# Kirkice/3DGaussian

Measured on AMD Instinct MI355X. Metric: Mpixels/sec fwd+bwd @1M Gaussians 800×800; PSNR vs torch ref, higher is better.
Workload: dtype f32 (splat contractions on v_mfma_f32_32x32x16_f16 with f32 accumulation; every operand in two round-to-nearest f16 pieces, pre-scaled into f16's normal range, three piece products: <= 3*2^-22 per product, forward and backward; no-depth-gradient mode)

## Files before the change

3dgaussian_amd/csrc/gr_hip.hip:

```cpp

#include <hip/hip_runtime.h>
#include <hipcub/hipcub.hpp>
#include <rocprim/rocprim.hpp>

#include <cmath>
#include <cstdint>
#include <cstdio>
#include <cstdlib>
#include <cstring>
#include <atomic>
#include <mutex>
#include <string>
#include <vector>

#include "../../include/gr_hip.h"

#ifndef GR_TAIL2
#define GR_TAIL2 1
#endif
#ifndef GR_DEBUG_PREP_REPS
#define GR_DEBUG_PREP_REPS 1
#endif
#ifndef GR_DEBUG_BIN_REPS
#define GR_DEBUG_BIN_REPS 1
#endif
#ifndef GR_DEBUG_SKIP
#define GR_DEBUG_SKIP 0
#endif

#define GR_VERSION_STR "gr_hip 0.1.0 (gfx950)"

namespace {

thread_local std::string g_last_error;

gr_status set_error(gr_status st, const std::string& msg) {
  g_last_error = msg;
  return st;
}

#define GR_HIP_TRY(expr)                                                                          \
  do {                                                                                            \
    hipError_t e_ = (expr);                                                                       \
    if (e_ != hipSuccess)                                                                         \
      return set_error(GR_ERR_HIP, std::string("HIP error: ") + hipGetErrorString(e_) + " (" +   \
// ... 190 lines not shown
  const float lox = (float)(tx * v.T) + 0.5f, hix = (float)xe + 0.5f;
  const float cx = px < lox ? lox : (px > hix ? hix : px);
  const float dx = cx - px;
  return (dx * dx) * qx;
}
__device__ __forceinline__ float tile_ey(const ViewK& v, float py, float qy, int ty) {
  const int ye = min(ty * v.T + v.T - 1, v.H - 1);
  const float loy = (float)(ty * v.T) + 0.5f, hiy = (float)ye + 0.5f;
  const float cy = py < loy ? loy : (py > hiy ? hiy : py);
  const float dy = cy - py;
  return (dy * dy) * qy;
}
__device__ __forceinline__ int tile_class_e(float e, float thr_cut, float thr_core) {
  return !(e >= thr_cut) ? 0 : (e >= thr_core ? 2 : 1);
}

__device__ __forceinline__ bool tile_pass(const ViewK& v, float px, float py, float qx, float qy, int tx, int ty) {
  return tile_emax(v, px, py, qx, qy, tx, ty) >= radius_thr(v.cutoff);
}

__device__ __forceinline__ int tile_class(const ViewK& v, float px, float py, float qx, float qy, int tx, int ty) {
  const float e = tile_emax(v, px, py, qx, qy, tx, ty);
  if (!(e >= radius_thr(v.cutoff))) return 0;
  return e >= radius_thr(v.core) ? 2 : 1;
}

__device__ __forceinline__ float qcoef(float s) { return (-0.5f * LOG2E) / (s * s); }


constexpr int REC4 = 2;
// ... 298 lines not shown
template <int CD>
__device__ __forceinline__ unsigned long long preprocess_vals(const ViewK& v, int i, float mx, float my, float mz, float s0,
                                                              float s1, const float* __restrict__ col, float op,
                                                              const Geom& g) {
  Proj p;
  project(v, mx, my, mz, s0, s1, p);
  float c[3];
  eval_color<CD>(v, mx, my, mz, col, c);
  int4 r;
  const float qx = qcoef(p.sx);
  const float qy = qcoef(p.sy);
  int core = 0, tail = 0;
  const int area = tile_rect(v, p, op, r);
  if (area > 0) {
    const float thr_cut = radius_thr(v.cutoff), thr_core = radius_thr(v.core);
    for (int ty = r.y; ty <= r.w; ++ty) {
      const float ey = tile_ey(v, p.py, qy, ty);
      for (int tx = r.x; tx <= r.z; ++tx) {
        const int cls = tile_class_e(tile_ex(v, p.px, qx, tx) + ey, thr_cut, thr_core);
        core += cls == 2;
        tail += cls == 1;
      }
    }
  }
  float4* rec = g.rec + (size_t)REC4 * i;
  rec[0] = make_float4(p.px, p.py, qx, qy);
  rec[1] = make_float4(op < 0.0f ? 0.0f : op, clamp01(c[0]), clamp01(c[1]), clamp01(c[2]));
  g.zr[i] = p.za;
  g.rect[i] = r;
  g.counts[i] = (unsigned long long)core | ((unsigned long long)tail << 32);
  return (unsigned long long)core | ((unsigned long long)tail << 32);
}

template <int CD>
__device__ __forceinline__ unsigned long long preprocess_one(const ViewK& v, int i, const float* __restrict__ means,
                                                             const float* __restrict__ scales,
// ... 180 lines not shown
  const Cnt2 cn{i < n ? counts[i].v : 0ull};
  const Cnt2 cb{bsum[b]};
  const int Kc = (int)offsets[n].c();
  const int4 rc = i < n ? rect[i] : make_int4(0, 0, -1, -1);
  const float4 a = i < n ? rec[(size_t)REC4 * i] : make_float4(0.f, 0.f, 0.f, 0.f);
  unsigned long long tot;
  const unsigned long long ex = block_exclusive_scan<4>(cn.v, wsum, tot);
  const int c0 = (int)cb.c(), t0 = (int)cb.t();
  const int nc = (int)(tot & 0xffffffffull), nt = (int)(tot >> 32);
  const bool staged = nc + nt <= EWIN_BLK;
  const unsigned long long run = cb.v + ex;
  if (i < n) offsets[i].v = run;
  if (cn.v != 0) {
    int kc = (int)(run & 0xffffffffull), kt = (int)(run >> 32);
    const float thr_cut = radius_thr(v.cutoff), thr_core = radius_thr(v.core);
    for (int ty = rc.y; ty <= rc.w; ++ty) {
      const float ey = tile_ey(v, a.y, a.w, ty);
      for (int tx = rc.x; tx <= rc.z; ++tx) {
        const int cls = tile_class_e(tile_ex(v, a.x, a.z, tx) + ey, thr_cut, thr_core);
        if (cls == 0) continue;
        const int t = ty * v.tiles_x + tx;
        const int e = cls == 2 ? kc++ - c0 : nc + (kt++ - t0);
        if (staged) {
          sK[e] = (uint16_t)t;
          sI[e] = i;
        } else {
          const int k = e < nc ? c0 + e : Kc + t0 + (e - nc);
          keys[k] = (uint16_t)t;
          ids[k] = i;
        }
      }
    }
  }
  if (!staged) return;
  __syncthreads();
  for (int e = tid; e < nc + nt; e += 256) {
    const int k = e < nc ? c0 + e : Kc + t0 + (e - nc);
    keys[k] = sK[e];
    ids[k] = sI[e];
  }
}
__global__ __launch_bounds__(256) void k_emit_offsets(ViewK v, int n, const int4* __restrict__ rect, const Cnt2* __restrict__ counts,
                                                      const unsigned long long* __restrict__ bsum, Cnt2* __restrict__ offsets,
                                                      const float4* __restrict__ rec, uint16_t* __restrict__ keys,
// ... 658 lines not shown
#ifndef GR_FWD_F16
#define GR_FWD_F16 1
#endif
#ifndef GR_F16_SA
#define GR_F16_SA 4
#endif
#ifndef GR_F16_SB
#define GR_F16_SB 12
#endif
__device__ __forceinline__ int f16_sa_of(float omax) {
  if (!(omax <= 3.0e38f)) return GR_F16_SA;
  int e = 0;
  (void)frexpf(omax, &e);
  return GR_F16_SA - (e > 11 ? e - 11 : 0);
}
__device__ __forceinline__ float f16_resid_lo(float x, unsigned h) {
  float r;
  asm("v_fma_mix_f32 %0, -%1, 1.0, %2 op_sel_hi:[1,0,0]" : "=v"(r) : "v"(h), "v"(x));
  return r;
}
__device__ __forceinline__ float f16_resid_hi(float x, unsigned h) {
  float r;
  asm("v_fma_mix_f32 %0, -%1, 1.0, %2 op_sel:[1,0,0] op_sel_hi:[1,0,0]" : "=v"(r) : "v"(h), "v"(x));
  return r;
}
typedef _Float16 f16x2h_t __attribute__((ext_vector_type(2)));
__device__ __forceinline__ unsigned pk_f16(float a, float b) {
  return __builtin_bit_cast(unsigned, __builtin_convertvector(f32x2_t{a, b}, f16x2h_t));
}
__device__ __forceinline__ void split2h_frag2(const f32x2_t (&v)[4], s16x8 (&f)[2]) {
  unsigned h[4], l[4];
#pragma unroll
  for (int p = 0; p < 4; ++p) {
    h[p] = pk_f16(v[p].x, v[p].y);
    l[p] = pk_f16(f16_resid_lo(v[p].x, h[p]), f16_resid_hi(v[p].y, h[p]));
  }
  f[0] = as_frag(make_uint4(h[0], h[1], h[2], h[3]));
  f[1] = as_frag(make_uint4(l[0], l[1], l[2], l[3]));
}
__device__ __forceinline__ void split2h_frag(const float (&v)[8], s16x8 (&f)[2]) {
  unsigned h[4], l[4];
#pragma unroll
  for (int p = 0; p < 4; ++p) {
    h[p] = pk_f16(v[2 * p], v[2 * p + 1]);
    l[p] = pk_f16(f16_resid_lo(v[2 * p], h[p]), f16_resid_hi(v[2 * p + 1], h[p]));
  }
  f[0] = as_frag(make_uint4(h[0], h[1], h[2], h[3]));
  f[1] = as_frag(make_uint4(l[0], l[1], l[2], l[3]));
}
__device__ __forceinline__ int f16_exp_of(float m) {
  if (!(m > 0.0f) || !(m <= 3.0e38f)) return 0;
  int e = 0;
  (void)frexpf(m, &e);
  return 14 - e;
}
typedef _Float16 f16x8_t __attribute__((ext_vector_type(8)));
__device__ __forceinline__ f32x4 mfma16h(const s16x8& a, const s16x8& b, f32x4 c) {
  return __builtin_amdgcn_mfma_f32_16x16x32_f16(__builtin_bit_cast(f16x8_t, a), __builtin_bit_cast(f16x8_t, b), c, 0, 0, 0);
}
__device__ __forceinline__ f32x4 mfma16h_split2(const s16x8 (&a)[2], const s16x8 (&b)[2], f32x4 c) {
  c = mfma16h(a[1], b[0], c);
  c = mfma16h(a[0], b[1], c);
  return mfma16h(a[0], b[0], c);
// ... 36 lines not shown

template <bool TAIL, bool PRECISE, bool ZCH = true>
__device__ __forceinline__ void fwd_accumulate_bf16(float* smem, int n, int k0, int k1, int tid, int wave, float xc, float yc,
                                                    int gq, const int* __restrict__ pairs, const float4* __restrict__ rec,
                                                    f32x4& cW, f32x4& cR, f32x4& cG, f32x4& cB, f32x4& cD, float sa) {
  constexpr int BUF = FWD_PLANES * TP;
  auto stage = [&](int g, int b) {
    glds4_planes<TAIL, ZCH>(rec_of(g, n, rec), zrec_of(g, n, rec), smem + b * BUF + 64 * wave);
  };
  stage(stage_pair(stage_id(k0 + tid, k1, pairs), k0 + tid, k1), 0);
  int idn = stage_id(k0 + TP + tid, k1, pairs);
  int buf = 0;
  const f32x2_t X = {xc, xc}, Y = {yc, yc};
  constexpr bool F16 = GR_FWD_F16 && !PRECISE && !TAIL && !ZCH;
  const f32x2_t SA = {sa, sa}, SB = {(float)GR_F16_SB, (float)GR_F16_SB};
  (void)SA;
  (void)SB;
  for (int base = k0; base < k1; base += TP, buf ^= 1) {
    stage_wait();
    GR_STAGE_SYNC();
    if (base + TP < k1) stage(stage_pair(idn, base + TP + tid, k1), buf ^ 1);
    idn = stage_id(base + 2 * TP + tid, k1, pairs);
    const int cnt = min(TP, k1 - base) - wave * 64;
    const int nst = cnt <= 0 ? 0 : min(2, (cnt + 31) >> 5);
    for (int st = 0; st < nst; ++st) {
      const float* s = smem + buf * BUF + wave * 64 + st * 32 + 8 * gq;
      auto ld = [&](int f, f32x2_t (&v)[4]) {
        const float4 u0 = *reinterpret_cast<const float4*>(s + f * TP);
        const float4 u1 = *reinterpret_cast<const float4*>(s + f * TP + 4);
        v[0] = f32x2_t{u0.x, u0.y};
        v[1] = f32x2_t{u0.z, u0.w};
        v[2] = f32x2_t{u1.x, u1.y};
// ... 21 lines not shown
        oe[p] = o[p] * ex;
        aW[p] = oe[p];
        if constexpr (ZCH) aD[p] = oe[p] * z[p];
      }
      s16x8 fb[3], f3[3], fb2h[2];
      if constexpr (PRECISE) {
        split3_frag2(bv, fb);
        split3_frag2(aW, f3);
        cW = mfma16_split3(f3, fb, cW);
        if constexpr (ZCH) {
          split3_frag2(aD, f3);
          cD = mfma16_split3(f3, fb, cD);
        }
      } else if (F16) {
        s16x8 f2[2];
        split2h_frag2(bv, fb2h);
        split2h_frag2(aW, f2);
        cW = mfma16h_split2(f2, fb2h, cW);
      } else {
        s16x8 f2b[2], f2[2];
        split2_frag2(bv, f2b);
        fb[0] = f2b[0];
        fb[1] = f2b[1];
        split2_frag2(aW, f2);
        cW = mfma16_split2<false>(f2, fb, cW);
        if constexpr (ZCH) {
          split2_frag2(aD, f2);
          cD = mfma16_split2<false>(f2, fb, cD);
        }
      }
      if constexpr (!TAIL) {
        f32x2_t c[4], a[4];
        s16x8 f2[2];
        if constexpr (F16) {
          ld(5, c);
#pragma unroll
          for (int p = 0; p < 4; ++p) a[p] = oe[p] * c[p];
          split2h_frag2(a, f2);
          cR = mfma16h_split2(f2, fb2h, cR);
          ld(6, c);
#pragma unroll
          for (int p = 0; p < 4; ++p) a[p] = oe[p] * c[p];
          split2h_frag2(a, f2);
          cG = mfma16h_split2(f2, fb2h, cG);
          ld(7, c);
#pragma unroll
          for (int p = 0; p < 4; ++p) a[p] = oe[p] * c[p];
          split2h_frag2(a, f2);
          cB = mfma16h_split2(f2, fb2h, cB);
        } else {
        ld(5, c);
#pragma unroll
        for (int p = 0; p < 4; ++p) a[p] = oe[p] * c[p];
        split2_frag2(a, f2);
        cR = mfma16_split2<PRECISE>(f2, fb, cR);
        ld(6, c);
#pragma unroll
        for (int p = 0; p < 4; ++p) a[p] = oe[p] * c[p];
        split2_frag2(a, f2);
        cG = mfma16_split2<PRECISE>(f2, fb, cG);
        ld(7, c);
#pragma unroll
        for (int p = 0; p < 4; ++p) a[p] = oe[p] * c[p];
// ... 80 lines not shown
      r[0][t] += r[0][t + w];
      r[1][t] += r[1][t + w];
      r[2][t] += r[2][t + w];
    }
    __syncthreads();
  }
  if (t != 0) return;
  float l = (float)(r[0][0] / (double)n1);
  if (n2 > 0) l = l + w_sil * (float)(r[1][0] / (double)n2);
  if (n3 > 0) l = l + w_depth * (float)(r[2][0] / (double)n3);
  *loss = l;
}

__device__ __forceinline__ float sign0(float t) { return t > 0.0f ? 1.0f : (t < 0.0f ? -1.0f : 0.0f); }

template <bool SSIM = false>
__device__ __forceinline__ void pixel_upstream(const ViewK& v, int p, float4 s, float Dp, const float* __restrict__ g_rgb,
                                               const float* __restrict__ g_alpha, const float* __restrict__ g_depth,
                                               const L1Args& l1, float (&u)[5], float& l_rgb, float& l_sil,
                                               const float* g_ssim = nullptr) {
  const float den = 1.0f + s.x, dden = s.x + 1e-6f;
  const float inv = 1.0f / den;
  float gW = 0.f;
  const float C[3] = {s.y, s.z, s.w};
  const float HWf = (float)v.W * (float)v.H;
#pragma unroll
  for (int k = 0; k < 3; ++k) {
    const float r = (view_bg(v, k) + C[k]) * inv;
    float gk;
    if (l1.t_rgb) {
      const float t = clamp01(r) - l1.t_rgb[3 * p + k];
      l_rgb += fabsf(t);
      if constexpr (SSIM)
        gk = sign0(t) * (((1.0f - l1.w_dssim) * l1.g_scale) / (3.0f * HWf)) + g_ssim[k];
      else
        gk = sign0(t) * (l1.g_scale / (3.0f * HWf));
    } else {
      gk = g_rgb[3 * p + k];
    }
    const float go = (r >= 0.0f && r <= 1.0f) ? gk : 0.0f;
    u[k] = go * inv;
    gW -= (go * r) * inv;
  }
  const float al = s.x * inv;
  float ga = 0.0f;
  bool has_a = g_alpha != nullptr;
  if (l1.t_rgb && l1.t_mask) {
    const float t = clamp01(al) - l1.t_mask[p];
    l_sil = fabsf(t);
    ga = sign0(t) * ((l1.w_sil * l1.g_scale) / HWf);
    has_a = true;
  } else if (g_alpha) {
    ga = g_alpha[p];
  }
  if (has_a && al >= 0.0f && al <= 1.0f) gW += ga * (inv * inv);
  const bool dfit = l1.t_rgb && l1.t_depth;
  if (g_depth || dfit) {
    const float d = Dp / dden;
    if (d >= 0.0f) {
      float gd;
      if (dfit) {
        const float M = l1.dscal[0], dm = M + 1e-6f;
        const float t = d / dm - l1.t_depth[p];
        gd = (sign0(t) * ((l1.w_depth * l1.g_scale) / HWf)) / dm;
        if (d == M) gd += l1.dscal[1];
      } else {
        gd = g_depth[p];
      }
      gW -= gd * Dp / (dden * dden);
      u[4] = gd / dden;
    }
  }
  u[3] = gW;
}

__device__ __forceinline__ float saved_depth(const float4* __restrict__ saved4, const float* __restrict__ savedD, int p) {
  const float d = savedD[p] / (saved4[p].x + 1e-6f);
  return d < 0.0f ? 0.0f : d;
}
// ... 187 lines not shown
  }
}

__device__ __forceinline__ void k_pixel_grads_body(ViewK v, const float4* __restrict__ saved4,
                                                     const float* __restrict__ savedD, const float* __restrict__ g_rgb,
                                                     const float* __restrict__ g_alpha, const float* __restrict__ g_depth,
                                                     uint4* __restrict__ UF, int pieces, L1Args l1, bool depth,
                                                     int* __restrict__ ticket, const BI blockIdx, const BI gridDim) {
  const int tile = blockIdx.x, tid = threadIdx.x;
  const int tx = tile % v.tiles_x, ty = tile / v.tiles_x;
  const int x = tx * T + (tid & (T - 1)), y = ty * T + (tid >> 4);
  float u[5] = {0.f, 0.f, 0.f, 0.f, 0.f};
  float l_rgb = 0.f, l_sil = 0.f;
  if (x < v.W && y < v.H) {
    const int p = y * v.W + x;
    pixel_upstream(v, p, saved4[p], savedD[p], g_rgb, g_alpha, g_depth, l1, u, l_rgb, l_sil);
  }
  if (l1.tile_loss) tile_loss_sums(tile, tid, l_rgb, l_sil, l1.tile_loss);
  __shared__ __attribute__((aligned(16))) float sU[6][TP];
  static_assert(sizeof(sU) >= 3 * 256 * sizeof(double), "tile_loss_total scratch");
#pragma unroll
  for (int k = 0; k < 5; ++k) sU[k][tid] = u[k];
  __syncthreads();
  tile_fragments(sU, reinterpret_cast<uint4*>(UF) + (size_t)tile * UF_FRAGS, tid, pieces, depth);
  if (l1.tile_loss && l1.loss_out) {
    __shared__ int last;
    const int tiles = v.tiles_x * v.tiles_y;
    if (arrive_last_tile(ticket, tiles, tile, &last))
      tile_loss_total<true>(l1.tile_loss, tiles, l1.n1, l1.n2, l1.w_sil, l1.t_depth ? l1.n1 / 3 : 0, l1.w_depth,
                            l1.loss_out, reinterpret_cast<double (*)[256]>(&sU[0][0]));
  }
// ... 20 lines not shown
};
__global__ __launch_bounds__(256) void k_pixel_grads_views(VBatch<k_pixel_grads_args> B) {
  const int vb = vbatch_view(B, (int)blockIdx.x);
  const k_pixel_grads_args& a = B.a[vb];
  const int lb = (int)blockIdx.x - B.first[vb], gx = B.gx[vb];
  k_pixel_grads_body(a.v, a.saved4, a.savedD, a.g_rgb, a.g_alpha, a.g_depth, a.UF, a.pieces, a.l1, a.depth, a.ticket, BI{lb % gx, lb / gx}, BI{gx, (B.first[vb + 1] - B.first[vb]) / gx});
}


__device__ __forceinline__ void l1_tile_epilogue(const ViewK& v, int tile, int tid, const float (&acc)[5], bool inside,
                                                 int p, const L1Args& l1, uint4* __restrict__ UF, float* lds,
                                                 bool fragments = true) {
  float u[5] = {0.f, 0.f, 0.f, 0.f, 0.f};
  float l_rgb = 0.f, l_sil = 0.f;
  if (inside)
    pixel_upstream(v, p, make_float4(acc[0], acc[1], acc[2], acc[3]), acc[4], nullptr, nullptr, nullptr, l1, u, l_rgb,
                   l_sil);
  tile_loss_sums(tile, tid, l_rgb, l_sil, l1.tile_loss);
  if (!fragments) return;
  float (*sU)[TP] = reinterpret_cast<float (*)[TP]>(lds);
#pragma unroll
  for (int k = 0; k < 4; ++k) sU[k][tid] = u[k];
  __syncthreads();
  tile_fragments(sU, UF + (size_t)tile * UF_FRAGS, tid, l1.pieces, false);
}

#ifndef GR_FWD_WAVES
#define GR_FWD_WAVES 5
#endif
#ifndef GR_FWD_WAVES3
#define GR_FWD_WAVES3 6
#endif
// ... 440 lines not shown
#define GR_BWD32_PHASE() __builtin_amdgcn_sched_barrier(0)
#else
#define GR_BWD32_PHASE() ((void)0)
#endif
constexpr int F32_PLANES = 8;
constexpr int F32_BUF = F32_PLANES * TP;
constexpr int F32_LD = T32 + 1;
__device__ __forceinline__ f32x16 mfma32h(const s16x8& a, const s16x8& b, f32x16 c) {
  return __builtin_amdgcn_mfma_f32_32x32x16_f16(__builtin_bit_cast(f16x8_t, a), __builtin_bit_cast(f16x8_t, b), c, 0, 0, 0);
}
__device__ __forceinline__ f32x16 mfma32b(const s16x8& a, const s16x8& b, f32x16 c) {
  return __builtin_amdgcn_mfma_f32_32x32x16_bf16(a, b, c, 0, 0, 0);
}
__device__ __forceinline__ constexpr int kslot_off(int j) { return j < 4 ? j : j + 4; }

__device__ __forceinline__ void k_fwd32_l1_body(ViewK v, int n, const int4* __restrict__ items,
                                                                 const int* __restrict__ num_items,
                                                                 const int2* __restrict__ ranges, const int* __restrict__ pairs,
                                                                 const float4* __restrict__ rec, float* __restrict__ fwd_part,
                                                                 float* __restrict__ out_rgb, float* __restrict__ out_alpha,
                                                                 L1Args l1, uint4* __restrict__ UF, const int* __restrict__ f16_sa,
                                                                 const int* __restrict__ tile_item0, int* __restrict__ ticket,
                                                                 int ch, const BI blockIdx, const BI gridDim) {
  __shared__ __attribute__((aligned(16))) float smem[4 * 2 * T32 * F32_LD];
  static_assert(sizeof(smem) >= 2 * F32_BUF * sizeof(float) && sizeof(smem) >= 3 * 256 * sizeof(double), "k_fwd32_l1 LDS");
  __shared__ int last_flag;
  const int nitems = num_items[0], nfull = num_items[1];
  if ((int)blockIdx.x >= nitems) return;
  const int item = (int)blockIdx.x < nfull ? xcd_item(blockIdx.x, nfull) : (int)blockIdx.x;
  const int4 it = items[item];
  const int tile = it.x >> 1, k0 = it.y, k1 = it.z;
  const int tx = tile % v.tiles_x, ty = tile / v.tiles_x;
  const int tid = threadIdx.x, wave = tid >> 6, lane = tid & 63, r = lane & 31, h = lane >> 5;
  const int sa = f16_sa ? *f16_sa : GR_F16_SA;
  f32x16 cW = {}, cR = {}, cG = {}, cB = {};
  if (k1 > k0) {
    auto stage = [&](int g, int b) { glds4_planes<false, false>(rec_of(g, n, rec), nullptr, smem + b * F32_BUF + 64 * wave); };
    stage(stage_pair(stage_id(k0 + tid, k1, pairs), k0 + tid, k1), 0);
    int idn = stage_id(k0 + TP + tid, k1, pairs);
    int buf = 0;
    const float xc = (float)(tx * T32 + r) + 0.5f, yc = (float)(ty * T32 + r) + 0.5f;
    const f32x2_t X = {xc, xc}, Y = {yc, yc}, SA = {(float)sa, (float)sa}, SB = {(float)GR_F16_SB, (float)GR_F16_SB};
    for (int base = k0; base < k1; base += TP, buf ^= 1) {
      stage_wait();
      if (base + TP < k1) stage(stage_pair(idn, base + TP + tid, k1), buf ^ 1);
      idn = stage_id(base + 2 * TP + tid, k1, pairs);
      const int cnt = min(TP, k1 - base) - wave * 64;
      const int nks = cnt <= 0 ? 0 : min(4, (cnt + 15) >> 4);
      for (int ks = 0; ks < nks; ++ks) {
        const float* s = smem + buf * F32_BUF + wave * 64 + ks * 16 + 4 * h;
        auto ld = [&](int f, f32x2_t (&q)[4]) {
          const float4 u0 = *reinterpret_cast<const float4*>(s + f * TP);
          const float4 u1 = *reinterpret_cast<const float4*>(s + f * TP + 8);
          q[0] = f32x2_t{u0.x, u0.y};
          q[1] = f32x2_t{u0.z, u0.w};
          q[2] = f32x2_t{u1.x, u1.y};
          q[3] = f32x2_t{u1.z, u1.w};
        };
        f32x2_t oe[4], bv[4];
        {
          f32x2_t px[4], qx[4], o[4];
          ld(0, px);
          ld(2, qx);
          ld(4, o);
#pragma unroll
          for (int p = 0; p < 4; ++p) {
            const f32x2_t dx = X - px[p];
            const f32x2_t ax = __builtin_elementwise_fma(dx * qx[p], dx, SA);
            const f32x2_t ex = {__builtin_amdgcn_exp2f(ax.x), __builtin_amdgcn_exp2f(ax.y)};
            oe[p] = o[p] * ex;
          }
        }
        __builtin_amdgcn_sched_barrier(0);
        {
          f32x2_t py[4], qy[4];
          ld(1, py);
          ld(3, qy);
#pragma unroll
          for (int p = 0; p < 4; ++p) {
            const f32x2_t dy = Y - py[p];
            const f32x2_t ay = __builtin_elementwise_fma(dy * qy[p], dy, SB);
            bv[p] = f32x2_t{__builtin_amdgcn_exp2f(ay.x), __builtin_amdgcn_exp2f(ay.y)};
          }
        }
        __builtin_amdgcn_sched_barrier(0);
        s16x8 fb[2], fa[2];
        split2h_frag2(bv, fb);
        split2h_frag2(oe, fa);
        cW = mfma32h(fa[1], fb[0], cW);
        cW = mfma32h(fa[0], fb[1], cW);
        cW = mfma32h(fa[0], fb[0], cW);
        f32x2_t c[4], a[4];
#define GR_FWD32_CH(F, ACC)                                   \
  ld(F, c);                                                   \
  _Pragma("unroll") for (int p = 0; p < 4; ++p) a[p] = oe[p] * c[p]; \
  split2h_frag2(a, fa);                                       \
  ACC = mfma32h(fa[1], fb[0], ACC);                           \
  ACC = mfma32h(fa[0], fb[1], ACC);                           \
  ACC = mfma32h(fa[0], fb[0], ACC);
        GR_FWD32_CH(5, cR)
        GR_FWD32_CH(6, cG)
        GR_FWD32_CH(7, cB)
#undef GR_FWD32_CH
      }
    }
    const float sc = __builtin_ldexpf(1.0f, -(sa + GR_F16_SB));
    cW *= sc;
    cR *= sc;
    cG *= sc;
    cB *= sc;
  }
// ... 35 lines not shown
#pragma unroll
      for (int c = 0; c < 4; ++c) acc[q][c] = 0.f;
    for (int e = 0; e < nch; ++e)
#pragma unroll
      for (int q = 0; q < 4; ++q) {
        const float4 pv = ld_through16(src, 4 * 4 * TP32 * e + 16 * (256 * q + tid));
        acc[q][0] += pv.x;
        acc[q][1] += pv.y;
        acc[q][2] += pv.z;
        acc[q][3] += pv.w;
      }
    if (tid == 0) ticket[tile] = 0;
  }
  float u[4][5];
  float l_rgb = 0.f, l_sil = 0.f;
#pragma unroll
  for (int q = 0; q < 4; ++q) {
    const int x = tx * T32 + px0, y = ty * T32 + py0 + 8 * q;
#pragma unroll
    for (int c = 0; c < 5; ++c) u[q][c] = 0.f;
    if (x < v.W && y < v.H && ty >= v.ty0 && ty < v.ty1) {
      const int p = y * v.W + x;
      const float a5[5] = {acc[q][0], acc[q][1], acc[q][2], acc[q][3], 0.0f};
      write_pixel(v, p, a5, out_rgb, out_alpha, nullptr, nullptr, nullptr);
      float lr = 0.f, ls = 0.f;
      pixel_upstream(v, p, make_float4(acc[q][0], acc[q][1], acc[q][2], acc[q][3]), 0.0f, nullptr, nullptr, nullptr, l1,
                     u[q], lr, ls);
      l_rgb += lr;
      l_sil += ls;
    }
  }
  tile_loss_sums(tile, tid, l_rgb, l_sil, l1.tile_loss);
  if (nch > 0) {
    float* sU = smem;
#pragma unroll
    for (int q = 0; q < 4; ++q)
#pragma unroll
      for (int c = 0; c < 4; ++c) sU[c * T32 * F32_LD + px0 * F32_LD + py0 + 8 * q] = u[q][c];
    __syncthreads();
    const float HWf = (float)v.W * (float)v.H, gC = fabsf(l1.g_scale) / (3.0f * HWf);
    const int eC = f16_exp_of(gC), eWb = f16_exp_of(3.0f * gC + fabsf(l1.w_sil * l1.g_scale) / HWf);
    const int ex4[4] = {eC, eC, eC, eWb};
    uint4* fr = UF + (size_t)tile * UF32_STRIDE;
    if (tid == 0) fr[UF32_FRAGS] = make_uint4((unsigned)ex4[0], (unsigned)ex4[1], (unsigned)ex4[2], (unsigned)ex4[3]);
    for (int e = tid; e < 16 * 64; e += 256) {
      const int set = e >> 6, l = e & 63, side = set >> 3, c = (set >> 1) & 3, s = set & 1;
      const int sc = c == 0 ? ex4[0] : (c == 1 ? ex4[1] : (c == 2 ? ex4[2] : ex4[3]));
      float val[8];
      const int m = l & 31, hh = l >> 5;
#pragma unroll
      for (int j = 0; j < 8; ++j) {
        const int k = 16 * s + kslot_pixel(hh, j);
        val[j] = ldexpf(side == 0 ? sU[c * T32 * F32_LD + k * F32_LD + m] : sU[c * T32 * F32_LD + m * F32_LD + k], sc);
      }
      s16x8 f2[2];
      split2h_frag(val, f2);
      __builtin_memcpy(&fr[(set * 2 + 0) * 64 + l], &f2[0], 16);
      __builtin_memcpy(&fr[(set * 2 + 1) * 64 + l], &f2[1], 16);
    }
  }
  const int tiles = v.tiles_x * v.tiles_y;
  if (arrive_last_tile(ticket, tiles, tile, &last_flag))
    tile_loss_total<true>(l1.tile_loss, tiles, l1.n1, l1.n2, l1.w_sil, 0, 0.0f, l1.loss_out,
                          reinterpret_cast<double (*)[256]>(smem));
}
__global__ __launch_bounds__(256, GR_FWD32_WAVES) void k_fwd32_l1(ViewK v, int n, const int4* __restrict__ items,
                                                                 const int* __restrict__ num_items,
                                                                 const int2* __restrict__ ranges, const int* __restrict__ pairs,
                                                                 const float4* __restrict__ rec, float* __restrict__ fwd_part,
                                                                 float* __restrict__ out_rgb, float* __restrict__ out_alpha,
                                                                 L1Args l1, uint4* __restrict__ UF, const int* __restrict__ f16_sa,
// ... 38 lines not shown
  __shared__ __attribute__((aligned(16))) uint4 sUF[2 * 4 * 2 * 2 * 64];
  const int nitems = num_items[1];
  if ((int)blockIdx.x >= nitems) return;
  const int item = xcd_item(blockIdx.x, nitems);
  const int4 it = items[item];
  const int tile = it.x >> 1, k0 = it.y, k1 = it.z;
  if (k1 <= k0) return;
  const int tx = tile % v.tiles_x, ty = tile / v.tiles_x;
  const int tid = threadIdx.x, wave = tid >> 6, lane = tid & 63, r = lane & 31, h = lane >> 5;
  {
    const uint4* src = UF + (size_t)tile * UF32_STRIDE;
    for (int cc = wave; cc < 32; cc += 4) glds16(src + 64 * cc + lane, sUF + 64 * cc);
  }
  const uint4 e4 = UF[(size_t)tile * UF32_STRIDE + UF32_FRAGS];
  const int eC0 = (int)e4.x, eC1 = (int)e4.y, eC2 = (int)e4.z, eW = (int)e4.w;
  const float pxb[2] = {(float)(tx * T32 + 4 * h) + 0.5f, (float)(tx * T32 + 16 + 4 * h) + 0.5f};
  const float pyb[2] = {(float)(ty * T32 + 4 * h) + 0.5f, (float)(ty * T32 + 16 + 4 * h) + 0.5f};
  {
    const int k = k0 + wave * WG + (lane < WG ? lane : 0);
    if (lane < WG) {
      const int gid = stage_pair(stage_id(k, k1, pairs), k, k1);
      glds16(rec_of(gid, n, rec), &sA[0][WG * wave]);
      glds16(rec_of(gid, n, rec) + 1, &sB[0][WG * wave]);
    }
  }
  int idn = stage_id(k0 + NB + wave * WG + (lane < WG ? lane : 0), k1, pairs);
  int buf = 0;
  for (int base = k0; base < k1; base += NB, buf ^= 1) {
    stage_wait();
    if (base == k0) __syncthreads();
// ... 31 lines not shown
      auto contract = [&](int side, int c, const s16x8 (&B)[2][2]) {
        const uint4* A0 = sUF + ((side * 4 + c) * 2 + 0) * 2 * 64;
        f32x16 d = {};
#pragma unroll
        for (int s = 0; s < 2; ++s) d = mfma32h(as_frag(A0[(s * 2 + 1) * 64 + lane]), B[s][0], d);
#pragma unroll
        for (int s = 0; s < 2; ++s) {
          const s16x8 a0 = as_frag(A0[(s * 2) * 64 + lane]);
          d = mfma32h(a0, B[s][1], d);
          d = mfma32h(a0, B[s][0], d);
        }
        return d;
      };
      const float4 bs = make_float4(b.x, ldexpf(b.y, eW - eC0), ldexpf(b.z, eW - eC1), ldexpf(b.w, eW - eC2));
      s16x8 BT[2][2], BR[2][2];
      split2h_frag(ex[0], BT[0]);
      split2h_frag(ex[1], BT[1]);
      float p[16];
      {
        const f32x16 D3 = contract(0, 3, BT);
#pragma unroll
        for (int i = 0; i < 16; ++i) p[i] = D3[i];
      }
      f32x16 Dc = contract(0, 0, BT);
      GR_BWD32_PHASE();
#pragma unroll
      for (int c = 0; c < 3; ++c) {
        const float bc = c == 0 ? bs.y : (c == 1 ? bs.z : bs.w);
        f32x16 Dn;
        if (c < 2) {
          Dn = contract(0, c + 1, BT);
        } else {
          split2h_frag(ey[0], BR[0]);
          split2h_frag(ey[1], BR[1]);
          Dn = contract(1, 3, BR);
        }
#pragma unroll
        for (int i = 0; i < 16; ++i) {
          S[c] = fmaf(ey[i >> 3][i & 7], Dc[i], S[c]);
          p[i] = fmaf(bc, Dc[i], p[i]);
        }
        if (c == 2) {
#pragma unroll
          for (int i = 0; i < 16; ++i) {
            const int s = i >> 3, q = i & 7;
            const float oq = (float)kslot_off(q);
            const float t = ey[s][q] * p[i];
            S4s[s] += t;
            if (q != 0) {
// ... 1206 lines not shown
    }
    sA[0][o] = a0;
    sA[1][o] = a1;
    sA[2][o] = a2;
  }
  __syncthreads();
  float u[5] = {0.f, 0.f, 0.f, 0.f, 0.f};
  float l_rgb = 0.f, l_sil = 0.f;
  if (inside) {
    const float scale = -((l1.w_dssim * l1.g_scale) / (3.0f * ((float)v.W * (float)v.H)));
    const int o = (tid >> 4) * TC + (tid & (T - 1)) * C;
    float gs[3];
#pragma unroll
    for (int k = 0; k < 3; ++k)
      gs[k] = scale * fmaf(tgt[k], sA[2][o + k], fmaf(2.0f * saved_colour(v, s, k), sA[1][o + k], sA[0][o + k]));
    pixel_upstream<true>(v, p, s, Dp, nullptr, nullptr, nullptr, l1, u, l_rgb, l_sil, gs);
  }
  tile_loss_sums(tile, tid, l_rgb, l_sil, l1.tile_loss);
  float (*sU)[TP] = reinterpret_cast<float (*)[TP]>(&tm[0][0]);
#pragma unroll
  for (int k = 0; k < 5; ++k) sU[k][tid] = u[k];
  __syncthreads();
  tile_fragments(sU, UF + (size_t)tile * UF_FRAGS, tid, pieces, depth);
  __shared__ int last;
  const int tiles = v.tiles_x * v.tiles_y;
  if (arrive_last_tile(ticket, tiles, tile, &last))
    tile_loss_total_ssim(l1.tile_loss, ssim_partial, tiles, l1.n1, l1.n2, l1.w_sil, l1.t_depth ? l1.n1 / 3 : 0, l1.w_depth,
                         l1.w_dssim, l1.loss_out, reinterpret_cast<double (*)[256]>(&tm[0][0]));
}

struct AccList {
// ... 1787 lines not shown
```

Measured before the change: 1558.

## Straight-line tile classify, restructure f16 split and fwd32 loops, hoist loss scales

For Gaussians whose tile rectangle is at most 3x3, tile classification in preprocess and emit now runs as a fully unrolled fixed-size pass instead of nested loops. The f16 residual split drops the inline v_fma_mix asm for plain fma against a device-global 'one' (gr_f16_unit), which keeps the compiler from folding it away. The fwd32 inner loop is regrouped into separate per-stage loops behind a packed/scalar switch. The upstream loss scale factors are hoisted out of the per-pixel path, and an extra GR_BWD32_PHASE is inserted in the backward pass. Together these aim to cut ALU and scheduling overhead, at the cost of an extra global load and changed instruction scheduling.

Result: no change. 1547 (-0.7%).

```diff
diff --git a/3dgaussian_amd/csrc/gr_hip.hip b/3dgaussian_amd/csrc/gr_hip.hip
--- a/3dgaussian_amd/csrc/gr_hip.hip
+++ b/3dgaussian_amd/csrc/gr_hip.hip
@@ -29,6 +29,8 @@
 #endif
 
 #define GR_VERSION_STR "gr_hip 0.1.0 (gfx950)"
+
+__device__ float gr_f16_unit = 1.0f;
 
 namespace {
 
@@ -249,6 +251,28 @@
 __device__ __forceinline__ int tile_class_e(float e, float thr_cut, float thr_core) {
   return !(e >= thr_cut) ? 0 : (e >= thr_core ? 2 : 1);
 }
+#ifndef GR_CLASSIFY_STRAIGHT
+#define GR_CLASSIFY_STRAIGHT 1
+#endif
+constexpr int RECT_SL = 3;
+__device__ __forceinline__ bool rect_straightline(const int4& r) {
+  return GR_CLASSIFY_STRAIGHT && r.z - r.x < RECT_SL && r.w - r.y < RECT_SL;
+}
+__device__ __forceinline__ void tile_class_rect3(const ViewK& v, float px, float py, float qx, float qy, const int4& r,
+                                                 float thr_cut, float thr_core, int (&cls)[RECT_SL * RECT_SL]) {
+  const int nx = r.z - r.x + 1, ny = r.w - r.y + 1;
+  float ex[RECT_SL], ey[RECT_SL];
+#pragma unroll
+  for (int j = 0; j < RECT_SL; ++j) {
+    ex[j] = tile_ex(v, px, qx, r.x + j);
+    ey[j] = tile_ey(v, py, qy, r.y + j);
+  }
+#pragma unroll
+  for (int jy = 0; jy < RECT_SL; ++jy)
+#pragma unroll
+    for (int jx = 0; jx < RECT_SL; ++jx)
+      cls[RECT_SL * jy + jx] = (jx < nx && jy < ny) ? tile_class_e(ex[jx] + ey[jy], thr_cut, thr_core) : 0;
+}
 
 __device__ __forceinline__ bool tile_pass(const ViewK& v, float px, float py, float qx, float qy, int tx, int ty) {
   return tile_emax(v, px, py, qx, qy, tx, ty) >= radius_thr(v.cutoff);
@@ -577,12 +601,22 @@
   const int area = tile_rect(v, p, op, r);
   if (area > 0) {
     const float thr_cut = radius_thr(v.cutoff), thr_core = radius_thr(v.core);
-    for (int ty = r.y; ty <= r.w; ++ty) {
-      const float ey = tile_ey(v, p.py, qy, ty);
-      for (int tx = r.x; tx <= r.z; ++tx) {
-        const int cls = tile_class_e(tile_ex(v, p.px, qx, tx) + ey, thr_cut, thr_core);
-        core += cls == 2;
-        tail += cls == 1;
+    if (rect_straightline(r)) {
+      int cls[RECT_SL * RECT_SL];
+      tile_class_rect3(v, p.px, p.py, qx, qy, r, thr_cut, thr_core, cls);
+#pragma unroll
+      for (int k = 0; k < RECT_SL * RECT_SL; ++k) {
+        core += cls[k] == 2;
+        tail += cls[k] == 1;
+      }
+    } else {
+      for (int ty = r.y; ty <= r.w; ++ty) {
+        const float ey = tile_ey(v, p.py, qy, ty);
+        for (int tx = r.x; tx <= r.z; ++tx) {
+          const int cls = tile_class_e(tile_ex(v, p.px, qx, tx) + ey, thr_cut, thr_core);
+          core += cls == 2;
+          tail += cls == 1;
+        }
       }
     }
   }
@@ -793,20 +827,32 @@
   if (cn.v != 0) {
     int kc = (int)(run & 0xffffffffull), kt = (int)(run >> 32);
     const float thr_cut = radius_thr(v.cutoff), thr_core = radius_thr(v.core);
-    for (int ty = rc.y; ty <= rc.w; ++ty) {
-      const float ey = tile_ey(v, a.y, a.w, ty);
-      for (int tx = rc.x; tx <= rc.z; ++tx) {
-        const int cls = tile_class_e(tile_ex(v, a.x, a.z, tx) + ey, thr_cut, thr_core);
-        if (cls == 0) continue;
-        const int t = ty * v.tiles_x + tx;
-        const int e = cls == 2 ? kc++ - c0 : nc + (kt++ - t0);
-        if (staged) {
-          sK[e] = (uint16_t)t;
-          sI[e] = i;
-        } else {
-          const int k = e < nc ? c0 + e : Kc + t0 + (e - nc);
-          keys[k] = (uint16_t)t;
-          ids[k] = i;
+    auto emit = [&](int cls, int tx, int ty) {
+      const int t = ty * v.tiles_x + tx;
+      const int e = cls == 2 ? kc++ - c0 : nc + (kt++ - t0);
+      if (staged) {
+        sK[e] = (uint16_t)t;
+        sI[e] = i;
+      } else {
+        const int k = e < nc ? c0 + e : Kc + t0 + (e - nc);
+        keys[k] = (uint16_t)t;
+        ids[k] = i;
+      }
+    };
+    if (rect_straightline(rc)) {
+      int cls[RECT_SL * RECT_SL];
+      tile_class_rect3(v, a.x, a.y, a.z, a.w, rc, thr_cut, thr_core, cls);
+#pragma unroll
+      for (int jy = 0; jy < RECT_SL; ++jy)
+#pragma unroll
+        for (int jx = 0; jx < RECT_SL; ++jx)
+          if (cls[RECT_SL * jy + jx] != 0) emit(cls[RECT_SL * jy + jx], rc.x + jx, rc.y + jy);
+    } else {
+      for (int ty = rc.y; ty <= rc.w; ++ty) {
+        const float ey = tile_ey(v, a.y, a.w, ty);
+        for (int tx = rc.x; tx <= rc.z; ++tx) {
+          const int cls = tile_class_e(tile_ex(v, a.x, a.z, tx) + ey, thr_cut, thr_core);
+          if (cls != 0) emit(cls, tx, ty);
         }
       }
     }
@@ -1495,39 +1541,47 @@
   (void)frexpf(omax, &e);
   return GR_F16_SA - (e > 11 ? e - 11 : 0);
 }
-__device__ __forceinline__ float f16_resid_lo(float x, unsigned h) {
-  float r;
-  asm("v_fma_mix_f32 %0, -%1, 1.0, %2 op_sel_hi:[1,0,0]" : "=v"(r) : "v"(h), "v"(x));
-  return r;
-}
-__device__ __forceinline__ float f16_resid_hi(float x, unsigned h) {
-  float r;
-  asm("v_fma_mix_f32 %0, -%1, 1.0, %2 op_sel:[1,0,0] op_sel_hi:[1,0,0]" : "=v"(r) : "v"(h), "v"(x));
-  return r;
-}
 typedef _Float16 f16x2h_t __attribute__((ext_vector_type(2)));
-__device__ __forceinline__ unsigned pk_f16(float a, float b) {
-  return __builtin_bit_cast(unsigned, __builtin_convertvector(f32x2_t{a, b}, f16x2h_t));
-}
-__device__ __forceinline__ void split2h_frag2(const f32x2_t (&v)[4], s16x8 (&f)[2]) {
-  unsigned h[4], l[4];
+__device__ __forceinline__ float f16_one() { return gr_f16_unit; }
+__device__ __forceinline__ float f16_resid_lo(float x, f16x2h_t h, float one) { return __builtin_fmaf(-(float)h.x, one, x); }
+__device__ __forceinline__ float f16_resid_hi(float x, f16x2h_t h, float one) { return __builtin_fmaf(-(float)h.y, one, x); }
+__device__ __forceinline__ f16x2h_t pk_f16(float a, float b) {
+  return __builtin_convertvector(f32x2_t{a, b}, f16x2h_t);
+}
+__device__ __forceinline__ unsigned f16x2_bits(f16x2h_t h) { return __builtin_bit_cast(unsigned, h); }
+template <bool ROUNDS>
+__device__ __forceinline__ void split2h_frag(const float (&v)[8], s16x8 (&f)[2], float one) {
+  f16x2h_t h[4], l[4];
+  if constexpr (ROUNDS) {
+    float r[8];
+#pragma unroll
+    for (int p = 0; p < 4; ++p) h[p] = pk_f16(v[2 * p], v[2 * p + 1]);
+#pragma unroll
+    for (int p = 0; p < 4; ++p) {
+      r[2 * p] = f16_resid_lo(v[2 * p], h[p], one);
+      r[2 * p + 1] = f16_resid_hi(v[2 * p + 1], h[p], one);
+    }
+#pragma unroll
+    for (int p = 0; p < 4; ++p) l[p] = pk_f16(r[2 * p], r[2 * p + 1]);
+  } else {
+#pragma unroll
+    for (int p = 0; p < 4; ++p) {
+      h[p] = pk_f16(v[2 * p], v[2 * p + 1]);
+      l[p] = pk_f16(f16_resid_lo(v[2 * p], h[p], one), f16_resid_hi(v[2 * p + 1], h[p], one));
+    }
+  }
+  f[0] = as_frag(make_uint4(f16x2_bits(h[0]), f16x2_bits(h[1]), f16x2_bits(h[2]), f16x2_bits(h[3])));
+  f[1] = as_frag(make_uint4(f16x2_bits(l[0]), f16x2_bits(l[1]), f16x2_bits(l[2]), f16x2_bits(l[3])));
+}
+template <bool ROUNDS>
+__device__ __forceinline__ void split2h_frag2(const f32x2_t (&v)[4], s16x8 (&f)[2], float one) {
+  float u[8];
 #pragma unroll
   for (int p = 0; p < 4; ++p) {
-    h[p] = pk_f16(v[p].x, v[p].y);
-    l[p] = pk_f16(f16_resid_lo(v[p].x, h[p]), f16_resid_hi(v[p].y, h[p]));
-  }
-  f[0] = as_frag(make_uint4(h[0], h[1], h[2], h[3]));
-  f[1] = as_frag(make_uint4(l[0], l[1], l[2], l[3]));
-}
-__device__ __forceinline__ void split2h_frag(const float (&v)[8], s16x8 (&f)[2]) {
-  unsigned h[4], l[4];
-#pragma unroll
-  for (int p = 0; p < 4; ++p) {
-    h[p] = pk_f16(v[2 * p], v[2 * p + 1]);
-    l[p] = pk_f16(f16_resid_lo(v[2 * p], h[p]), f16_resid_hi(v[2 * p + 1], h[p]));
-  }
-  f[0] = as_frag(make_uint4(h[0], h[1], h[2], h[3]));
-  f[1] = as_frag(make_uint4(l[0], l[1], l[2], l[3]));
+    u[2 * p] = v[p].x;
+    u[2 * p + 1] = v[p].y;
+  }
+  split2h_frag<ROUNDS>(u, f, one);
 }
 __device__ __forceinline__ int f16_exp_of(float m) {
   if (!(m > 0.0f) || !(m <= 3.0e38f)) return 0;
@@ -1594,8 +1648,10 @@
   const f32x2_t X = {xc, xc}, Y = {yc, yc};
   constexpr bool F16 = GR_FWD_F16 && !PRECISE && !TAIL && !ZCH;
   const f32x2_t SA = {sa, sa}, SB = {(float)GR_F16_SB, (float)GR_F16_SB};
+  const float one = F16 ? f16_one() : 1.0f;
   (void)SA;
   (void)SB;
+  (void)one;
   for (int base = k0; base < k1; base += TP, buf ^= 1) {
     stage_wait();
     GR_STAGE_SYNC();
@@ -1647,8 +1703,8 @@
         }
       } else if (F16) {
         s16x8 f2[2];
-        split2h_frag2(bv, fb2h);
-        split2h_frag2(aW, f2);
+        split2h_frag2<false>(bv, fb2h, one);
+        split2h_frag2<false>(aW, f2, one);
         cW = mfma16h_split2(f2, fb2h, cW);
       } else {
         s16x8 f2b[2], f2[2];
@@ -1669,17 +1725,17 @@
           ld(5, c);
 #pragma unroll
           for (int p = 0; p < 4; ++p) a[p] = oe[p] * c[p];
-          split2h_frag2(a, f2);
+          split2h_frag2<false>(a, f2, one);
           cR = mfma16h_split2(f2, fb2h, cR);
           ld(6, c);
 #pragma unroll
           for (int p = 0; p < 4; ++p) a[p] = oe[p] * c[p];
-          split2h_frag2(a, f2);
+          split2h_frag2<false>(a, f2, one);
           cG = mfma16h_split2(f2, fb2h, cG);
           ld(7, c);
 #pragma unroll
           for (int p = 0; p < 4; ++p) a[p] = oe[p] * c[p];
-          split2h_frag2(a, f2);
+          split2h_frag2<false>(a, f2, one);
           cB = mfma16h_split2(f2, fb2h, cB);
         } else {
         ld(5, c);
@@ -1790,16 +1846,34 @@
 
 __device__ __forceinline__ float sign0(float t) { return t > 0.0f ? 1.0f : (t < 0.0f ? -1.0f : 0.0f); }
 
+struct UpScale {
+  float rgb;
+  float sil;
+  float depth;
+};
+template <bool SSIM = false>
+__device__ __forceinline__ UpScale upstream_scales(const ViewK& v, const L1Args& l1) {
+  UpScale us = {0.0f, 0.0f, 0.0f};
+  if (!l1.t_rgb) return us;
+  const float HWf = (float)v.W * (float)v.H;
+  if constexpr (SSIM)
+    us.rgb = ((1.0f - l1.w_dssim) * l1.g_scale) / (3.0f * HWf);
+  else
+    us.rgb = l1.g_scale / (3.0f * HWf);
+  us.sil = (l1.w_sil * l1.g_scale) / HWf;
+  us.depth = (l1.w_depth * l1.g_scale) / HWf;
+  return us;
+}
+
 template <bool SSIM = false>
 __device__ __forceinline__ void pixel_upstream(const ViewK& v, int p, float4 s, float Dp, const float* __restrict__ g_rgb,
                                                const float* __restrict__ g_alpha, const float* __restrict__ g_depth,
-                                               const L1Args& l1, float (&u)[5], float& l_rgb, float& l_sil,
-                                               const float* g_ssim = nullptr) {
+                                               const L1Args& l1, const UpScale& us, float (&u)[5], float& l_rgb,
+                                               float& l_sil, const float* g_ssim = nullptr) {
   const float den = 1.0f + s.x, dden = s.x + 1e-6f;
   const float inv = 1.0f / den;
   float gW = 0.f;
   const float C[3] = {s.y, s.z, s.w};
-  const float HWf = (float)v.W * (float)v.H;
 #pragma unroll
   for (int k = 0; k < 3; ++k) {
     const float r = (view_bg(v, k) + C[k]) * inv;
@@ -1808,9 +1882,9 @@
       const float t = clamp01(r) - l1.t_rgb[3 * p + k];
       l_rgb += fabsf(t);
       if constexpr (SSIM)
-        gk = sign0(t) * (((1.0f - l1.w_dssim) * l1.g_scale) / (3.0f * HWf)) + g_ssim[k];
+        gk = sign0(t) * us.rgb + g_ssim[k];
       else
-        gk = sign0(t) * (l1.g_scale / (3.0f * HWf));
+        gk = sign0(t) * us.rgb;
     } else {
       gk = g_rgb[3 * p + k];
     }
@@ -1824,7 +1898,7 @@
   if (l1.t_rgb && l1.t_mask) {
     const float t = clamp01(al) - l1.t_mask[p];
     l_sil = fabsf(t);
-    ga = sign0(t) * ((l1.w_sil * l1.g_scale) / HWf);
+    ga = sign0(t) * us.sil;
     has_a = true;
   } else if (g_alpha) {
     ga = g_alpha[p];
@@ -1838,7 +1912,7 @@
       if (dfit) {
         const float M = l1.dscal[0], dm = M + 1e-6f;
         const float t = d / dm - l1.t_depth[p];
-        gd = (sign0(t) * ((l1.w_depth * l1.g_scale) / HWf)) / dm;
+        gd = (sign0(t) * us.depth) / dm;
         if (d == M) gd += l1.dscal[1];
       } else {
         gd = g_depth[p];
@@ -2056,7 +2130,7 @@
   float l_rgb = 0.f, l_sil = 0.f;
   if (x < v.W && y < v.H) {
     const int p = y * v.W + x;
-    pixel_upstream(v, p, saved4[p], savedD[p], g_rgb, g_alpha, g_depth, l1, u, l_rgb, l_sil);
+    pixel_upstream(v, p, saved4[p], savedD[p], g_rgb, g_alpha, g_depth, l1, upstream_scales(v, l1), u, l_rgb, l_sil);
   }
   if (l1.tile_loss) tile_loss_sums(tile, tid, l_rgb, l_sil, l1.tile_loss);
   __shared__ __attribute__((aligned(16))) float sU[6][TP];
@@ -2107,8 +2181,8 @@
   float u[5] = {0.f, 0.f, 0.f, 0.f, 0.f};
   float l_rgb = 0.f, l_sil = 0.f;
   if (inside)
-    pixel_upstream(v, p, make_float4(acc[0], acc[1], acc[2], acc[3]), acc[4], nullptr, nullptr, nullptr, l1, u, l_rgb,
-                   l_sil);
+    pixel_upstream(v, p, make_float4(acc[0], acc[1], acc[2], acc[3]), acc[4], nullptr, nullptr, nullptr, l1,
+                   upstream_scales(v, l1), u, l_rgb, l_sil);
   tile_loss_sums(tile, tid, l_rgb, l_sil, l1.tile_loss);
   if (!fragments) return;
   float (*sU)[TP] = reinterpret_cast<float (*)[TP]>(lds);
@@ -2579,6 +2653,33 @@
 }
 __device__ __forceinline__ constexpr int kslot_off(int j) { return j < 4 ? j : j + 4; }
 
+#ifndef GR_FWD32_PACKED
+#define GR_FWD32_PACKED 1
+#endif
+#if GR_FWD32_PACKED
+typedef f32x2_t fwd32_t;
+constexpr int FWD32_NV = 4;
+__device__ __forceinline__ fwd32_t fwd32_splat(float x) { return f32x2_t{x, x}; }
+__device__ __forceinline__ fwd32_t fwd32_exp2(fwd32_t a) { return f32x2_t{__builtin_amdgcn_exp2f(a.x), __builtin_amdgcn_exp2f(a.y)}; }
+__device__ __forceinline__ void fwd32_load(float4 u0, float4 u1, fwd32_t (&q)[4]) {
+  q[0] = f32x2_t{u0.x, u0.y};
+  q[1] = f32x2_t{u0.z, u0.w};
+  q[2] = f32x2_t{u1.x, u1.y};
+  q[3] = f32x2_t{u1.z, u1.w};
+}
+__device__ __forceinline__ void fwd32_split(const fwd32_t (&v)[4], s16x8 (&f)[2], float one) { split2h_frag2<true>(v, f, one); }
+#else
+typedef float fwd32_t;
+constexpr int FWD32_NV = 8;
+__device__ __forceinline__ fwd32_t fwd32_splat(float x) { return x; }
+__device__ __forceinline__ fwd32_t fwd32_exp2(fwd32_t a) { return __builtin_amdgcn_exp2f(a); }
+__device__ __forceinline__ void fwd32_load(float4 u0, float4 u1, fwd32_t (&q)[8]) {
+  q[0] = u0.x, q[1] = u0.y, q[2] = u0.z, q[3] = u0.w;
+  q[4] = u1.x, q[5] = u1.y, q[6] = u1.z, q[7] = u1.w;
+}
+__device__ __forceinline__ void fwd32_split(const fwd32_t (&v)[8], s16x8 (&f)[2], float one) { split2h_frag<true>(v, f, one); }
+#endif
+
 __device__ __forceinline__ void k_fwd32_l1_body(ViewK v, int n, const int4* __restrict__ items,
                                                                  const int* __restrict__ num_items,
                                                                  const int2* __restrict__ ranges, const int* __restrict__ pairs,
@@ -2598,6 +2699,7 @@
   const int tx = tile % v.tiles_x, ty = tile / v.tiles_x;
   const int tid = threadIdx.x, wave = tid >> 6, lane = tid & 63, r = lane & 31, h = lane >> 5;
   const int sa = f16_sa ? *f16_sa : GR_F16_SA;
+  const float one = f16_one();
   f32x16 cW = {}, cR = {}, cG = {}, cB = {};
   if (k1 > k0) {
     auto stage = [&](int g, int b) { glds4_planes<false, false>(rec_of(g, n, rec), nullptr, smem + b * F32_BUF + 64 * wave); };
@@ -2605,7 +2707,8 @@
     int idn = stage_id(k0 + TP + tid, k1, pairs);
     int buf = 0;
     const float xc = (float)(tx * T32 + r) + 0.5f, yc = (float)(ty * T32 + r) + 0.5f;
-    const f32x2_t X = {xc, xc}, Y = {yc, yc}, SA = {(float)sa, (float)sa}, SB = {(float)GR_F16_SB, (float)GR_F16_SB};
+    const fwd32_t X = fwd32_splat(xc), Y = fwd32_splat(yc), SA = fwd32_splat((float)sa), SB = fwd32_splat((float)GR_F16_SB);
+    constexpr int NV = FWD32_NV;
     for (int base = k0; base < k1; base += TP, buf ^= 1) {
       stage_wait();
       if (base + TP < k1) stage(stage_pair(idn, base + TP + tid, k1), buf ^ 1);
@@ -2614,52 +2717,50 @@
       const int nks = cnt <= 0 ? 0 : min(4, (cnt + 15) >> 4);
       for (int ks = 0; ks < nks; ++ks) {
         const float* s = smem + buf * F32_BUF + wave * 64 + ks * 16 + 4 * h;
-        auto ld = [&](int f, f32x2_t (&q)[4]) {
-          const float4 u0 = *reinterpret_cast<const float4*>(s + f * TP);
-          const float4 u1 = *reinterpret_cast<const float4*>(s + f * TP + 8);
-          q[0] = f32x2_t{u0.x, u0.y};
-          q[1] = f32x2_t{u0.z, u0.w};
-          q[2] = f32x2_t{u1.x, u1.y};
-          q[3] = f32x2_t{u1.z, u1.w};
+        auto ld = [&](int f, fwd32_t (&q)[NV]) {
+          fwd32_load(*reinterpret_cast<const float4*>(s + f * TP), *reinterpret_cast<const float4*>(s + f * TP + 8), q);
         };
-        f32x2_t oe[4], bv[4];
+        fwd32_t oe[NV], bv[NV];
         {
-          f32x2_t px[4], qx[4], o[4];
+          fwd32_t px[NV], qx[NV], o[NV], d[NV], a[NV];
           ld(0, px);
           ld(2, qx);
           ld(4, o);
 #pragma unroll
-          for (int p = 0; p < 4; ++p) {
-            const f32x2_t dx = X - px[p];
-            const f32x2_t ax = __builtin_elementwise_fma(dx * qx[p], dx, SA);
-            const f32x2_t ex = {__builtin_amdgcn_exp2f(ax.x), __builtin_amdgcn_exp2f(ax.y)};
-            oe[p] = o[p] * ex;
-          }
+          for (int p = 0; p < NV; ++p) d[p] = X - px[p];
+#pragma unroll
+          for (int p = 0; p < NV; ++p) a[p] = d[p] * qx[p];
+#pragma unroll
+          for (int p = 0; p < NV; ++p) a[p] = __builtin_elementwise_fma(a[p], d[p], SA);
+#pragma unroll
+          for (int p = 0; p < NV; ++p) oe[p] = o[p] * fwd32_exp2(a[p]);
         }
         __builtin_amdgcn_sched_barrier(0);
         {
-          f32x2_t py[4], qy[4];
+          fwd32_t py[NV], qy[NV], d[NV], a[NV];
           ld(1, py);
           ld(3, qy);
 #pragma unroll
-          for (int p = 0; p < 4; ++p) {
-            const f32x2_t dy = Y - py[p];
-            const f32x2_t ay = __builtin_elementwise_fma(dy * qy[p], dy, SB);
-            bv[p] = f32x2_t{__builtin_amdgcn_exp2f(ay.x), __builtin_amdgcn_exp2f(ay.y)};
-          }
+          for (int p = 0; p < NV; ++p) d[p] = Y - py[p];
+#pragma unroll
+          for (int p = 0; p < NV; ++p) a[p] = d[p] * qy[p];
+#pragma unroll
+          for (int p = 0; p < NV; ++p) a[p] = __builtin_elementwise_fma(a[p], d[p], SB);
+#pragma unroll
+          for (int p = 0; p < NV; ++p) bv[p] = fwd32_exp2(a[p]);
         }
         __builtin_amdgcn_sched_barrier(0);
         s16x8 fb[2], fa[2];
-        split2h_frag2(bv, fb);
-        split2h_frag2(oe, fa);
+        fwd32_split(bv, fb, one);
+        fwd32_split(oe, fa, one);
         cW = mfma32h(fa[1], fb[0], cW);
         cW = mfma32h(fa[0], fb[1], cW);
         cW = mfma32h(fa[0], fb[0], cW);
-        f32x2_t c[4], a[4];
+        fwd32_t c[NV], a[NV];
 #define GR_FWD32_CH(F, ACC)                                   \
   ld(F, c);                                                   \
-  _Pragma("unroll") for (int p = 0; p < 4; ++p) a[p] = oe[p] * c[p]; \
-  split2h_frag2(a, fa);                                       \
+  _Pragma("unroll") for (int p = 0; p < NV; ++p) a[p] = oe[p] * c[p]; \
+  fwd32_split(a, fa, one);                                    \
   ACC = mfma32h(fa[1], fb[0], ACC);                           \
   ACC = mfma32h(fa[0], fb[1], ACC);                           \
   ACC = mfma32h(fa[0], fb[0], ACC);
@@ -2725,6 +2826,7 @@
   }
   float u[4][5];
   float l_rgb = 0.f, l_sil = 0.f;
+  const UpScale us = upstream_scales(v, l1);
 #pragma unroll
   for (int q = 0; q < 4; ++q) {
     const int x = tx * T32 + px0, y = ty * T32 + py0 + 8 * q;
@@ -2736,7 +2838,7 @@
       write_pixel(v, p, a5, out_rgb, out_alpha, nullptr, nullptr, nullptr);
       float lr = 0.f, ls = 0.f;
       pixel_upstream(v, p, make_float4(acc[q][0], acc[q][1], acc[q][2], acc[q][3]), 0.0f, nullptr, nullptr, nullptr, l1,
-                     u[q], lr, ls);
+                     us, u[q], lr, ls);
       l_rgb += lr;
       l_sil += ls;
     }
@@ -2765,7 +2867,7 @@
         val[j] = ldexpf(side == 0 ? sU[c * T32 * F32_LD + k * F32_LD + m] : sU[c * T32 * F32_LD + m * F32_LD + k], sc);
       }
       s16x8 f2[2];
-      split2h_frag(val, f2);
+      split2h_frag<false>(val, f2, one);
       __builtin_memcpy(&fr[(set * 2 + 0) * 64 + l], &f2[0], 16);
       __builtin_memcpy(&fr[(set * 2 + 1) * 64 + l], &f2[1], 16);
     }
@@ -2834,6 +2936,7 @@
   }
   const uint4 e4 = UF[(size_t)tile * UF32_STRIDE + UF32_FRAGS];
   const int eC0 = (int)e4.x, eC1 = (int)e4.y, eC2 = (int)e4.z, eW = (int)e4.w;
+  const float one = f16_one();
   const float pxb[2] = {(float)(tx * T32 + 4 * h) + 0.5f, (float)(tx * T32 + 16 + 4 * h) + 0.5f};
   const float pyb[2] = {(float)(ty * T32 + 4 * h) + 0.5f, (float)(ty * T32 + 16 + 4 * h) + 0.5f};
   {
@@ -2895,8 +2998,9 @@
       };
       const float4 bs = make_float4(b.x, ldexpf(b.y, eW - eC0), ldexpf(b.z, eW - eC1), ldexpf(b.w, eW - eC2));
       s16x8 BT[2][2], BR[2][2];
-      split2h_frag(ex[0], BT[0]);
-      split2h_frag(ex[1], BT[1]);
+      split2h_frag<false>(ex[0], BT[0], one);
+      split2h_frag<false>(ex[1], BT[1], one);
+      GR_BWD32_PHASE();
       float p[16];
       {
         const f32x16 D3 = contract(0, 3, BT);
@@ -2912,8 +3016,8 @@
         if (c < 2) {
           Dn = contract(0, c + 1, BT);
         } else {
-          split2h_frag(ey[0], BR[0]);
-          split2h_frag(ey[1], BR[1]);
+          split2h_frag<false>(ey[0], BR[0], one);
+          split2h_frag<false>(ey[1], BR[1], one);
           Dn = contract(1, 3, BR);
         }
 #pragma unroll
@@ -4150,7 +4254,7 @@
 #pragma unroll
     for (int k = 0; k < 3; ++k)
       gs[k] = scale * fmaf(tgt[k], sA[2][o + k], fmaf(2.0f * saved_colour(v, s, k), sA[1][o + k], sA[0][o + k]));
-    pixel_upstream<true>(v, p, s, Dp, nullptr, nullptr, nullptr, l1, u, l_rgb, l_sil, gs);
+    pixel_upstream<true>(v, p, s, Dp, nullptr, nullptr, nullptr, l1, upstream_scales<true>(v, l1), u, l_rgb, l_sil, gs);
   }
   tile_loss_sums(tile, tid, l_rgb, l_sil, l1.tile_loss);
   float (*sU)[TP] = reinterpret_cast<float (*)[TP]>(&tm[0][0]);
```
